# qasimyu/scssim

Hardware: AMD Instinct MI355X
Metric: paired-end read pairs/s (whole genreads job: MALBAC amplification + read allocation + read generation + FASTQ files, PE150 30x) (higher is better)
Workload: dtype u8/u32 (integer draws, byte sequences; fp64 only in the GC-weight draw and the allocation sums)

## Files before the change

include/scssim_hip.h:

```cpp
#ifndef SCSSIM_HIP_H
#define SCSSIM_HIP_H

#include <stddef.h>
#include <stdint.h>

#ifdef __cplusplus
extern "C" {
#endif

#define SCS_OK          0
#define SCS_EINVAL      1
#define SCS_EIO         2
#define SCS_EDEVICE     3
#define SCS_EOVERFLOW   4

typedef struct scs_ctx scs_ctx;

typedef struct scs_config {
    int      device;
    void*    stream;
    uint64_t seed;
    long     primers;
    double   gamma;
    double   coverage;
// ... 170 lines not shown
int         scs_profile_open(const char* profile_path, int paired, int isize, void** handle, char* errbuf, size_t errlen);
int         scs_profile_table(void* handle, int which, const uint32_t** thr, const double** cdf, size_t* n);
int         scs_profile_scalars(void* handle, double* out);
void        scs_profile_close(void* handle);

int         scs_fasta_probe(const char* fasta_path, int* n_records, uint64_t* total_bases, uint64_t* checksum,
                            char* names_buf, size_t names_len, char* errbuf, size_t errlen);
int         scs_simuvars_probe(const char* ref_fasta, const char* snp_file, const char* var_file, int* n_records, uint64_t* total_bases,
                               uint64_t* checksum, char* errbuf, size_t errlen);
int         scs_devbuf_probe(int device, uint64_t first_bytes, uint64_t second_bytes, uint64_t* caps, int* in_place);
int         scs_bgzf_probe(const void* text, uint64_t nbytes, uint32_t lds_out_cap, void* out, uint64_t cap, uint64_t* n_out);
int         scs_batch_plan_probe(uint64_t pairs, uint32_t read_length, int to_sink, int writers, int regions, int batch_shift,
                                 uint64_t* batch, uint32_t* nbatch, uint32_t* order, uint32_t* region_of, uint32_t cap);
int         scs_bgzf_device_probe(int device, const void* text, uint64_t nbytes, uint32_t zbase, void* out, uint64_t cap, uint64_t* n_out, int* guards_ok);
int         scs_scan_probe(int device, const uint32_t* in0, uint64_t n0, const uint32_t* in1, uint64_t n1, uint32_t* out0, uint32_t* out1);
int         scs_live_resources(uint64_t out[4]);
int         scs_fasta_write_index(const char* fasta_path, char* errbuf, size_t errlen);

int         scs_kernel_time(const scs_ctx* ctx, int which, const char** name, uint64_t* launches, double* ms, uint64_t* units);
int         scs_set_kernel_timing(scs_ctx* ctx, unsigned mask, unsigned every);

#ifdef __cplusplus
}
#endif
#endif
```

scssim_amd/csrc/scs_device.h:

```cpp
#pragma once
#include <stdint.h>
#include <hip/hip_runtime.h>
#include "scs_common.h"
#include "scs_simuvars.h"

namespace scs {

struct DevFrags {
    const uint64_t* goff;
    const uint32_t* len;
    const int8_t*   strand;
    const uint32_t* primers;
    uint32_t n;
    uint64_t gidx_base;
    const uint8_t* has_n;
};

struct DevAmps {
    uint32_t* parent;
    uint32_t* sl;
    uint16_t* gc;
    uint16_t* primers;
    uint64_t* uid;
    uint64_t* errs;
// ... 64 lines not shown
    int64_t  base; uint32_t flags;
    int32_t  k1;
    uint64_t e1, e2, uid;
};

void launch_attach_frags(hipStream_t s, const uint8_t* g, DevFrags fr, const uint32_t* slot_off, uint32_t* slots,
                         uint32_t* slot_tmpl, uint32_t* valid, const unsigned long long* primer_cut, uint32_t* primer_delta,
                         unsigned long long* len_part, AmplifyParams p, uint32_t t_first, uint32_t t_end, int undo, const unsigned long long* t_from);
void launch_frag_len_sum(hipStream_t s, const unsigned long long* len_part, uint32_t nf, unsigned long long* len_sum);
void launch_poisson(hipStream_t s, DevFrags fr, DevAmps semis, uint32_t n_semis, PoissonParams p, uint32_t* budget_f, uint32_t* budget_s,
                    unsigned long long* sums, unsigned long long* part, uint32_t* flags);
void launch_alloc_bpack(hipStream_t s, const double* w, const AllocPlan& pl, double* send);
void launch_alloc_bgather(hipStream_t s, const double* w, const AllocPlan& pl, const double* gathered, double* brow, int* bmap);
void launch_alloc_chunk_sum(hipStream_t s, const double* w, const double* brow, const AllocPlan& pl, double* part);
void launch_tree_sum(hipStream_t s, const double* part, uint32_t nch, double* scratch, double* total);
void launch_alloc_norm(hipStream_t s, double* w, double* brow, const int* bmap, const AllocPlan& pl, const double* total, unsigned long long reads,
                       uint32_t* rn, double* tp, uint32_t* crn, unsigned long long* sum_rn);
void launch_alloc_quota(hipStream_t s, const double* tp, uint32_t nch, unsigned long long reads, const unsigned long long* sum_rn, unsigned long long* sum_quota,
                        uint32_t* quota, double* probs, double* scratch, RngKey key);
void launch_alloc_sample(hipStream_t s, const double* w, const double* brow, const int* bmap, const AllocPlan& pl, const double* tp, const uint32_t* quota, RngKey key, uint32_t* rn);
void launch_alloc_odd_scan(hipStream_t s, const uint32_t* rn, uint32_t ac, uint32_t* odd_before, void* temp, size_t temp_bytes);
void launch_alloc_odd_counts(hipStream_t s, const uint32_t* odd_before, const AllocPlan& pl, unsigned long long* table);
void launch_alloc_parity(hipStream_t s, uint32_t* rn, const uint32_t* odd_before, uint32_t ac, const AllocPlan& pl, const unsigned long long* table);
void launch_attach_semis(hipStream_t s, const uint8_t* g, DevFrags fr, DevAmps semis, uint32_t n_semis, DevErrPool spool,
                         const uint32_t* slot_off, uint32_t* slots, uint32_t* slot_tmpl, uint32_t* valid,
                         const unsigned long long* primer_cut, uint32_t* primer_delta, AmplifyParams p, uint32_t t_first, uint32_t t_end, int undo, const unsigned long long* t_from);
uint32_t attach_dense_waves(uint32_t n_slots);
void launch_attach_plan(hipStream_t s, const uint32_t* slot_off, uint32_t nt, uint32_t n_slots, uint32_t* item_tmpl, uint32_t* wave_first, uint32_t* valid);
void launch_attach_dense(hipStream_t s, const uint8_t* g, DevFrags fr, DevAmps semis, DevErrPool spool, const uint32_t* slot_off, uint32_t* slots, const uint32_t* item_tmpl,
                         const uint32_t* wave_first, uint32_t n_slots, uint32_t* valid, const unsigned long long* primer_cut, uint32_t* primer_delta, AmplifyParams p, int undo,
                         const unsigned long long* t_from);
void launch_stock_check(hipStream_t s, const int64_t* cnt, const uint32_t* taken, unsigned long long* cut, bool from_frag, unsigned long long* info);
void launch_stock_list(hipStream_t s, const int64_t* cnt, const uint32_t* taken, uint32_t* eidx, uint32_t* etype, uint32_t* estart, unsigned long long* info);
void launch_stock_collect(hipStream_t s, const uint8_t* g, DevFrags fr, DevAmps semis, DevErrPool spool, bool from_frag, const uint32_t* slot_off, const uint32_t* slots,
                          const uint32_t* valid, const uint32_t* eidx, unsigned long long* list, unsigned long long* info, uint32_t t_first, uint32_t t_end);
// ... 148 lines not shown
```

scssim_amd/csrc/scs_k_allocate.hip:

```cpp
#include <utility>
#include <type_traits>
#include "scs_device.h"
#include "scs_seams.h"

#include <algorithm>
#include <cstdlib>
#include <cstring>
#include <rocprim/rocprim.hpp>
#include "scs_kernels_common.h"

namespace scs {

struct GcDraw { double y, r2; bool in; };
__device__ __forceinline__ GcDraw gc_attempt(uint32_t wx, uint32_t wy) {
    const double x = 2.0 * (((double)wx + 0.5) / 4294967296.0) - 1.0;
    const double y = 2.0 * (((double)wy + 0.5) / 4294967296.0) - 1.0;
    const double r2 = x * x + y * y;
    return GcDraw{y, r2, !(r2 > 1.0 || r2 == 0.0)};
}
__device__ __forceinline__ double gc_value(double mean, double sd, double y, double r2) {
    const double mult = __dsqrt_rn(-2.0 * det_log(r2) / r2);
    return mean + sd * (y * mult);
}
constexpr int WEIGHTS_BLOCK = 1024;
// ... 111 lines not shown
    double acc = 0;
    for (uint32_t i = lane; i < r.n; i += WAVE) acc += v[i];
    acc = wave_butterfly_f64(acc);
    if (lane == 0 && r.owner) part[r.c] = acc;
}
__global__ void __launch_bounds__(256) k_tree1000(const double* __restrict__ in, uint32_t n, double* __restrict__ out) {
    const uint32_t gq = blockIdx.x * 4 + (threadIdx.x >> 6), lane = threadIdx.x & 63;
    const uint32_t b = gq * ALLOC_CHUNK;
    if (b >= n) return;
    const uint32_t m = min(ALLOC_CHUNK, n - b);
    double acc = 0;
    for (uint32_t i = lane; i < m; i += WAVE) acc += in[b + i];
    acc = wave_butterfly_f64(acc);
    if (lane == 0) out[gq] = acc;
}
__global__ void __launch_bounds__(256) k_alloc_norm(double* __restrict__ w, double* __restrict__ brow, const int* __restrict__ bmap, AllocPlan pl,
                                                    const double* __restrict__ total, unsigned long long reads, uint32_t* __restrict__ rn,
                                                    double* __restrict__ tp, uint32_t* __restrict__ crn) {
    const uint32_t q = blockIdx.x * 4 + (threadIdx.x >> 6), lane = threadIdx.x & 63;
    if (q >= pl.n_interior + pl.n_boundary) return;
    const ChunkRef r = chunk_ref(pl, q);
    double* __restrict__ v = r.brow < 0 ? w + r.local0 : brow + (size_t)r.brow * ALLOC_CHUNK;
    const int* __restrict__ mp = r.brow < 0 ? nullptr : bmap + (size_t)r.brow * ALLOC_CHUNK;
    const double den = 2.2204e-16 + *total;
    double acc = 0; uint32_t cs = 0;
    for (uint32_t i = lane; i < r.n; i += WAVE) {
        const double p = v[i] / den;
        v[i] = p; acc += p;
        const uint32_t c = (uint32_t)(p * (double)(long long)reads);
        if (mp) { const int li = mp[i]; if (li >= 0) { rn[li] = c; cs += c; } }
        else { rn[r.local0 + i] = c; cs += c; }
    }
    acc = wave_butterfly_f64(acc);
    cs = wave_sum(cs);
    if (lane == 0) { if (r.owner) tp[r.c] = acc; crn[q] = cs; }
}
__global__ void __launch_bounds__(1024) k_sum_u32(const uint32_t* __restrict__ v, uint32_t n, unsigned long long* __restrict__ dst, int add) {
    __shared__ unsigned long long s_p[16];
    unsigned long long acc = 0;
    for (uint32_t i = threadIdx.x; i < n; i += blockDim.x) acc += v[i];
    acc = wave_sum_u64(acc);
    if ((threadIdx.x & 63) == 0) s_p[threadIdx.x >> 6] = acc;
    __syncthreads();
    if (threadIdx.x == 0) { unsigned long long t = 0; for (int k = 0; k < 16; ++k) t += s_p[k]; *dst = add ? *dst + t : t; }
}
__global__ void __launch_bounds__(256) k_alloc_quota(const double* __restrict__ tp, uint32_t nch, unsigned long long reads, const unsigned long long* __restrict__ sum_rn,
                                                     uint32_t* __restrict__ quota) {
    const uint32_t c = blockIdx.x * blockDim.x + threadIdx.x;
    if (c >= nch) return;
    const unsigned long long nres = reads - *sum_rn;
    quota[c] = (uint32_t)(tp[c] * (double)nres);
}
__global__ void __launch_bounds__(64) k_scan1000(const double* __restrict__ in, uint32_t n, double* __restrict__ out, double* __restrict__ last) {
    const uint32_t g = blockIdx.x, b = g * ALLOC_CHUNK, m = min(ALLOC_CHUNK, n - b), lane = threadIdx.x;
    double carry = 0;
    for (uint32_t r = 0; r < m; r += WAVE) {
        double s = r + lane < m ? in[b + r + lane] : 0.0;
#pragma unroll
        for (int d = 1; d < WAVE; d <<= 1) { const double t = shfl_up_f64(s, d); if ((int)lane >= d) s = s + t; }
// ... 10 lines not shown
__device__ __forceinline__ uint32_t first_le(const double* __restrict__ cdf, uint32_t n, double r) {
    uint32_t lo = 0, hi = n;
    while (lo < hi) { const uint32_t mid = (lo + hi) >> 1; if (r <= cdf[mid]) hi = mid; else lo = mid + 1; }
    return lo < n ? lo : n - 1;
}
__global__ void k_alloc_top_draws(const double* __restrict__ probs, uint32_t nch, unsigned long long reads, const unsigned long long* __restrict__ sum_rn,
                                  const unsigned long long* __restrict__ sum_quota, RngKey key, uint32_t* __restrict__ quota) {
    const uint32_t t = blockIdx.x * blockDim.x + threadIdx.x;
    const unsigned long long n = reads - *sum_rn - *sum_quota;
    if (t >= n) return;
    const U4 d = draw4(key, ST_ALLOC_TOP, 0, 0, t);
    const double r = 2.2204e-16 + (1 - 2.2204e-16) * ((double)d.w[0] / 4294967296.0);
    atomicAdd(&quota[first_le(probs, nch, r)], 1u);
}
__global__ void __launch_bounds__(256) k_alloc_sample(const double* __restrict__ w, const double* __restrict__ brow, const int* __restrict__ bmap, AllocPlan pl,
                                                      const double* __restrict__ tp, const uint32_t* __restrict__ quota, RngKey key, uint32_t* __restrict__ rn) {
    constexpr int ROUNDS = (ALLOC_CHUNK + WAVE - 1) / WAVE, WAVES = 4, MINE = ROUNDS / WAVES;
    static_assert(ROUNDS % WAVES == 0, "rounds of scan1000 divide among the waves");
    __shared__ double s_cdf[ALLOC_CHUNK];
    __shared__ uint32_t s_cnt[ALLOC_CHUNK];
    __shared__ double s_tot[ROUNDS];
    const uint32_t q = blockIdx.x, tid = threadIdx.x, lane = tid & 63u, wv = tid >> 6;
    const ChunkRef r = chunk_ref(pl, q);
    const uint32_t nq = quota[r.c];
    if (nq == 0) return;
    const double* __restrict__ v = r.brow < 0 ? w + r.local0 : brow + (size_t)r.brow * ALLOC_CHUNK;
    const double t = tp[r.c];
    double pv[MINE];
#pragma unroll
    for (int m = 0; m < MINE; ++m) { const uint32_t i = (uint32_t)((wv + WAVES * m) * WAVE) + lane; pv[m] = i < r.n ? v[i] : 0.0; }
#pragma unroll
    for (int m = 0; m < MINE; ++m) {
        const uint32_t k = wv + WAVES * m, i = k * WAVE + lane;
        double s = i < r.n ? pv[m] / t : 0.0;
#pragma unroll
        for (int d = 1; d < WAVE; d <<= 1) { const double u = shfl_up_f64(s, d); if ((int)lane >= d) s = s + u; }
        pv[m] = s;
        if (lane == 63) s_tot[k] = s;
    }
    __syncthreads();
#pragma unroll
    for (int m = 0; m < MINE; ++m) {
        const uint32_t k = wv + WAVES * m, i = k * WAVE + lane;
        double carry = 0;
        for (uint32_t z = 0; z < k; ++z) carry = carry + s_tot[z];
// ... 2 lines not shown
    __syncthreads();
    for (uint32_t j = tid; 4u * j < nq; j += blockDim.x) {
        const U4 d = draw4(key, ST_ALLOC_CHUNK, 0, r.c, j);
        double x[4]; uint32_t lo[4], hi[4];
#pragma unroll
        for (int i = 0; i < 4; ++i) { x[i] = 2.2204e-16 + (1 - 2.2204e-16) * ((double)d.w[i] / 4294967296.0); lo[i] = 0; hi[i] = r.n; }
        for (uint32_t span = r.n; span; span >>= 1) {
#pragma unroll
            for (int i = 0; i < 4; ++i)
                if (lo[i] < hi[i]) { const uint32_t mid = (lo[i] + hi[i]) >> 1; if (x[i] <= s_cdf[mid]) hi[i] = mid; else lo[i] = mid + 1; }
        }
#pragma unroll
        for (int i = 0; i < 4; ++i) if (4u * j + (uint32_t)i < nq) atomicAdd(&s_cnt[lo[i] < r.n ? lo[i] : r.n - 1], 1u);
    }
    __syncthreads();
    for (uint32_t i = tid; i < r.n; i += blockDim.x) {
        const uint32_t c = s_cnt[i];
        if (!c) continue;
        if (r.brow < 0) rn[r.local0 + i] += c;
        else { const int li = bmap[(size_t)r.brow * ALLOC_CHUNK + i]; if (li >= 0) rn[li] += c; }
    }
}
__global__ void k_alloc_odd_counts(const uint32_t* __restrict__ odd_before, AllocPlan pl, unsigned long long* __restrict__ table) {
    const uint32_t slot = threadIdx.x;
    if (slot >= ALLOC_SLOTS) return;
    const uint32_t n = pl.my_seg[slot].n, lo = pl.my_seg[slot].lo;
    table[(size_t)pl.my_seg[slot].order] = n ? odd_before[lo + n] - odd_before[lo] : 0u;
}
__global__ void __launch_bounds__(256) k_alloc_parity(uint32_t* __restrict__ rn, const uint32_t* __restrict__ odd_before, uint32_t ac, AllocPlan pl,
                                                      const unsigned long long* __restrict__ table) {
    __shared__ unsigned long long s_base[ALLOC_SLOTS];
    if (threadIdx.x < ALLOC_SLOTS) {
        unsigned long long b = 0;
        if (table) { const uint32_t ord = pl.my_seg[threadIdx.x].order; for (uint32_t k = 0; k < ord; ++k) b += table[k]; }
        s_base[threadIdx.x] = b;
// ... 24 lines not shown
void launch_alloc_chunk_sum(hipStream_t s, const double* w, const double* brow, const AllocPlan& pl, double* part) {
    const uint32_t nq = pl.n_interior + pl.n_boundary;
    if (nq) hipLaunchKernelGGL(k_alloc_chunk_sum, dim3(cdiv(nq, 4)), dim3(256), 0, s, w, brow, pl, part);
}
void launch_tree_sum(hipStream_t s, const double* part, uint32_t nch, double* scratch, double* total) {
    if (nch == 0) { (void)hipMemsetAsync(total, 0, 8, s); return; }
    if (nch == 1) { (void)hipMemcpyAsync(total, part, 8, hipMemcpyDeviceToDevice, s); return; }
    const double* cur = part; uint32_t n = nch; double* nxt = scratch;
    while (n > 1) {
        const uint32_t ng = cdiv(n, ALLOC_CHUNK);
        double* dst = ng == 1 ? total : nxt;
        hipLaunchKernelGGL(k_tree1000, dim3(cdiv(ng, 4)), dim3(256), 0, s, cur, n, dst);
        cur = dst; nxt += ng; n = ng;
    }
}
void launch_alloc_norm(hipStream_t s, double* w, double* brow, const int* bmap, const AllocPlan& pl, const double* total, unsigned long long reads,
                       uint32_t* rn, double* tp, uint32_t* crn, unsigned long long* sum_rn) {
    const uint32_t nq = pl.n_interior + pl.n_boundary;
    if (nq) hipLaunchKernelGGL(k_alloc_norm, dim3(cdiv(nq, 4)), dim3(256), 0, s, w, brow, bmap, pl, total, reads, rn, tp, crn);
    hipLaunchKernelGGL(k_sum_u32, dim3(1), dim3(1024), 0, s, crn, nq, sum_rn, 0);
}
static void scan_all_dev(hipStream_t s, const double* in, uint32_t n, double* out, double* scratch) {
    const uint32_t ng = cdiv(n, ALLOC_CHUNK);
    double* last = scratch; double* pre = scratch + ng;
    hipLaunchKernelGGL(k_scan1000, dim3(ng), dim3(64), 0, s, in, n, out, ng > 1 ? last : (double*)nullptr);
    if (ng == 1) return;
    scan_all_dev(s, last, ng, pre, scratch + 2 * (size_t)ng);
    hipLaunchKernelGGL(k_scan_fix, dim3(cdiv(n, 256)), dim3(256), 0, s, out, n, pre);
}
void launch_alloc_quota(hipStream_t s, const double* tp, uint32_t nch, unsigned long long reads, const unsigned long long* sum_rn, unsigned long long* sum_quota,
                        uint32_t* quota, double* probs, double* scratch, RngKey key) {
    if (nch == 0) return;
    hipLaunchKernelGGL(k_alloc_quota, dim3(cdiv(nch, 256)), dim3(256), 0, s, tp, nch, reads, sum_rn, quota);
    hipLaunchKernelGGL(k_sum_u32, dim3(1), dim3(1024), 0, s, quota, nch, sum_quota, 0);
    scan_all_dev(s, tp, nch, probs, scratch);
    hipLaunchKernelGGL(k_alloc_top_draws, dim3(cdiv((uint64_t)nch + 1024, 256)), dim3(256), 0, s, probs, nch, reads, sum_rn, sum_quota, key, quota);
}
void launch_alloc_sample(hipStream_t s, const double* w, const double* brow, const int* bmap, const AllocPlan& pl, const double* tp, const uint32_t* quota, RngKey key, uint32_t* rn) {
    const uint32_t nq = pl.n_interior + pl.n_boundary;
    if (nq) hipLaunchKernelGGL(k_alloc_sample, dim3(nq), dim3(256), 0, s, w, brow, bmap, pl, tp, quota, key, rn);
}
void launch_alloc_odd_scan(hipStream_t s, const uint32_t* rn, uint32_t ac, uint32_t* odd_before, void* temp, size_t temp_bytes) {
    (void)rocprim::exclusive_scan(temp, temp_bytes, rocprim::make_transform_iterator(rn, OddBit()), odd_before, 0u, (size_t)ac + 1, rocprim::plus<uint32_t>(), s);
}
void launch_alloc_odd_counts(hipStream_t s, const uint32_t* odd_before, const AllocPlan& pl, unsigned long long* table) {
    hipLaunchKernelGGL(k_alloc_odd_counts, dim3(1), dim3(64), 0, s, odd_before, pl, table);
}
void launch_alloc_parity(hipStream_t s, uint32_t* rn, const uint32_t* odd_before, uint32_t ac, const AllocPlan& pl, const unsigned long long* table) {
    if (ac) hipLaunchKernelGGL(k_alloc_parity, dim3(cdiv(ac, 256)), dim3(256), 0, s, rn, odd_before, ac, pl, table);
}
void launch_weights(hipStream_t s, DevAmps fulls, uint32_t n, DevTables tb, RngKey key, uint32_t frag_size, double* w) {
    if (n == 0) return;
    hipLaunchKernelGGL(k_weights, dim3(cdiv(n, (uint32_t)WEIGHTS_BLOCK)), dim3(WEIGHTS_BLOCK), 0, s, fulls, n, tb, key, frag_size, w);
}
using ScanCfg = rocprim::scan_config<256, 16, rocprim::block_load_method::block_load_transpose, rocprim::block_store_method::block_store_transpose, rocprim::block_scan_algorithm::using_warp_scan>;
// ... 38 lines not shown
```

scssim_amd/csrc/scs_k_amplify.hip:

```cpp
#include <utility>
#include <type_traits>
#include "scs_device.h"
#include "scs_seams.h"

#include <algorithm>
#include <cstdlib>
#include <cstring>
#include <rocprim/rocprim.hpp>
#include "scs_kernels_common.h"

namespace scs {
#ifdef SCS_PHASE_CLOCK
__device__ unsigned long long g_phase_att[8 * 256];
#endif
__global__ void k_amplify_init(int64_t* __restrict__ cnt, unsigned long long* __restrict__ cut, int64_t copies, uint32_t* __restrict__ delta, uint32_t* __restrict__ gdelta, uint32_t* __restrict__ flags,
                               unsigned long long* __restrict__ sums, unsigned long long nf_all, unsigned long long frag_len_all, unsigned long long total_primers,
                               uint32_t* __restrict__ pool_head_a, uint32_t* __restrict__ pool_head_b) {
    const uint32_t i = blockIdx.x * blockDim.x + threadIdx.x;
    if (i < 65536) { cnt[i] = copies; cut[i] = copies > 0 ? ~0ull : 0ull; delta[i] = 0; if (gdelta) gdelta[i] = 0; }
    if (i < SHARD_TAIL_WORDS && gdelta) gdelta[65536 + i] = 0;
    if (i < 16) sums[i] = i == DS_G_PRIMERS ? total_primers : i == DS_G_TOTALS || i == DS_G_NF ? nf_all : i == DS_G_TOTALS + 1 || i == DS_G_FRAG_LEN ? frag_len_all : i == DS_MIN_STOCK ? (unsigned long long)copies : 0ull;
    if (i == 0) { flags[0] = 0; if (pool_head_a) *pool_head_a = 0; if (pool_head_b) *pool_head_b = 0; }
}
__device__ __forceinline__ void stock_update(uint32_t i, int64_t* __restrict__ cnt, const uint32_t* __restrict__ taken, uint32_t* __restrict__ delta, unsigned long long* __restrict__ cut,
// ... 256 lines not shown
        }
        __syncthreads();
        if (!s_more) break;
    }
    if (tid == 0) {
        budget_f[t] = (uint32_t)(int)x; part[blockIdx.x] = (unsigned long long)x;
        if ((unsigned long long)x >= (1ull << 20)) atomicOr(flags, (uint32_t)FLAG_KEYSPACE);
    }
}

__global__ void __launch_bounds__(256) k_poisson(DevFrags fr, DevAmps semis, uint32_t n_cap, PoissonParams p, uint32_t* __restrict__ budget_f,
                                                 uint32_t* __restrict__ budget_s, unsigned long long* __restrict__ part, uint32_t* __restrict__ flags) {
    if (blockIdx.x < fr.n) poisson_frag_block(blockIdx.x, fr, p, budget_f, part, flags);
    else poisson_semis_block(blockIdx.x - fr.n, semis, n_cap, p, budget_s, part);
}
__global__ void __launch_bounds__(1024) k_sum_u64_add(const unsigned long long* __restrict__ v, uint32_t n, unsigned long long* __restrict__ dst) {
    __shared__ unsigned long long s_p[16];
    unsigned long long a = 0;
    for (uint32_t i = blockIdx.x * blockDim.x + threadIdx.x; i < n; i += gridDim.x * blockDim.x) a += v[i];
    a = wave_sum_u64(a);
    if ((threadIdx.x & 63) == 0) s_p[threadIdx.x >> 6] = a;
    __syncthreads();
    if (threadIdx.x == 0) { unsigned long long t = 0; for (int k = 0; k < 16; ++k) t += s_p[k]; if (t) atomicAdd(dst, t); }
}
__global__ void __launch_bounds__(1024) k_poisson_sums(const unsigned long long* __restrict__ part, uint32_t nf, uint32_t nb, unsigned long long* __restrict__ sums) {
    __shared__ unsigned long long s_p[2][16];
    unsigned long long a = 0, b = 0;
    for (uint32_t i = threadIdx.x; i < nb; i += blockDim.x) { const unsigned long long v = part[i]; if (i < nf) a += v; else b += v; }
    a = wave_sum_u64(a); b = wave_sum_u64(b);
    if ((threadIdx.x & 63) == 0) { s_p[0][threadIdx.x >> 6] = a; s_p[1][threadIdx.x >> 6] = b; }
    __syncthreads();
    if (threadIdx.x < 2) { unsigned long long t = 0; for (int k = 0; k < 16; ++k) t += s_p[threadIdx.x][k]; sums[threadIdx.x] += t; }
}

#define STOCK_KEY_BITS 46
template <bool FROM_FRAG> __device__ __forceinline__ unsigned long long attach_key(uint32_t t, uint32_t i) {
    return (((unsigned long long)t << (FROM_FRAG ? 20 : 12)) | i) + 1ull;
}
__global__ void __launch_bounds__(256) k_stock_check(const int64_t* __restrict__ cnt, const uint32_t* __restrict__ taken, unsigned long long* __restrict__ cut, int key_shift,
                                                     unsigned long long* __restrict__ info) {
    const uint32_t x = blockIdx.x * blockDim.x + threadIdx.x;
    if (x >= 65536u) return;
    const int64_t c = cnt[x]; const uint32_t d = taken[x];
    if ((int64_t)d > c) { atomicAdd(&info[0], 1ull); atomicAdd(&info[1], (unsigned long long)d); }
    else { const unsigned long long q = cut[x]; if (q != 0ull && q != ~0ull && (int64_t)d < c) { atomicAdd(&info[2], 1ull); atomicMax(&info[3], 0xFFFFFFFFull - ((q - 1ull) >> key_shift)); cut[x] = ~0ull; } }
}
__global__ void __launch_bounds__(1024) k_stock_list(const int64_t* __restrict__ cnt, const uint32_t* __restrict__ taken,
                                                     uint32_t* __restrict__ eidx, uint32_t* __restrict__ etype, uint32_t* __restrict__ estart, unsigned long long* __restrict__ info) {
// ... 354 lines not shown
    }
#ifdef SCS_PHASE_CLOCK
    __builtin_amdgcn_wave_barrier();
    if (lane < 8) atomicAdd(&g_phase_att[lane * 256 + (blockIdx.x & 255u)], lane == 7 ? 1ull : s_att_acc[lane]);
#endif
}

void launch_attach_frags(hipStream_t s, const uint8_t* g, DevFrags fr, const uint32_t* slot_off, uint32_t* slots, uint32_t* slot_tmpl,
                         uint32_t* valid, const unsigned long long* primer_cut, uint32_t* primer_delta, unsigned long long* len_part, AmplifyParams p,
                         uint32_t t_first, uint32_t t_end, int undo, const unsigned long long* t_from) {
    if (t_end <= t_first) return;
    DevAmps none{}; DevErrPool np{};
    hipLaunchKernelGGL((k_attach<true, 64>), dim3(t_end - t_first), dim3(64), 0, s, g, fr, none, 0u, np, slot_off, slots, slot_tmpl, valid, primer_cut, primer_delta, len_part, p, t_first, t_end, undo, t_from);
}
void launch_frag_len_sum(hipStream_t s, const unsigned long long* len_part, uint32_t nf, unsigned long long* len_sum) {
    if (nf) hipLaunchKernelGGL(k_sum_u64_add, dim3(std::min(cdiv(nf, 2048), 128u)), dim3(1024), 0, s, len_part, nf, len_sum);
}
void launch_poisson(hipStream_t s, DevFrags fr, DevAmps semis, uint32_t n_semis, PoissonParams p, uint32_t* budget_f, uint32_t* budget_s,
                    unsigned long long* sums, unsigned long long* part, uint32_t* flags) {
    const uint32_t semi_blocks = n_semis ? cdiv((uint64_t)n_semis + 1, 256) : 0u;
    if (fr.n + semi_blocks) {
        hipLaunchKernelGGL(k_poisson, dim3(fr.n + semi_blocks), dim3(256), 0, s, fr, semis, n_semis, p, budget_f, budget_s, part, flags);
        hipLaunchKernelGGL(k_poisson_sums, dim3(1), dim3(1024), 0, s, part, fr.n, fr.n + semi_blocks, sums);
    }
}
static int attach_semi_group(uint32_t n_semis) {
    static const int forced = seam_env("SCS_ATTACH_G") ? atoi(seam_env("SCS_ATTACH_G")) : 0;
    return forced == 2 || forced == 4 || forced == 8 || forced == 16 ? forced : (n_semis >= (1u << 18) ? 4 : 8);
}
uint32_t attach_dense_waves(uint32_t n_slots) { return n_slots / ATTACH_DENSE_STRIDE + 1u; }
void launch_attach_plan(hipStream_t s, const uint32_t* slot_off, uint32_t nt, uint32_t n_slots, uint32_t* item_tmpl, uint32_t* wave_first, uint32_t* valid) {
    hipLaunchKernelGGL(k_attach_plan, dim3(cdiv((uint64_t)nt + 1, 256)), dim3(256), 0, s, slot_off, nt, n_slots, attach_dense_waves(n_slots), item_tmpl, wave_first, valid);
}
void launch_attach_dense(hipStream_t s, const uint8_t* g, DevFrags fr, DevAmps semis, DevErrPool spool, const uint32_t* slot_off, uint32_t* slots, const uint32_t* item_tmpl,
                         const uint32_t* wave_first, uint32_t n_slots, uint32_t* valid, const unsigned long long* primer_cut, uint32_t* primer_delta, AmplifyParams p, int undo,
                         const unsigned long long* t_from) {
    const uint32_t row_words = (p.amp_max > p.amp_min ? (p.amp_max - p.amp_min) / 32u : 0u) + 2u;
    hipLaunchKernelGGL(k_attach_dense, dim3(attach_dense_waves(n_slots)), dim3(64), 0, s, g, fr, semis, spool, slot_off, slots, item_tmpl, wave_first, valid, primer_cut, primer_delta, p, 0u,
// ... 96 lines not shown
```

scssim_amd/csrc/scs_probes.cpp:

```cpp
#include "scs_ctx.h"
#include "scs_amp.h"
#include "scs_site.h"
#include "scs_support.h"

static int truth_probe(bool bam, int paired, int is_read2, uint32_t amp, uint32_t cnt, const char* rname, int n,
                       int64_t pos0, int reverse, const int32_t* events, int nev,
                       int64_t mate_pos0, int mate_reverse, const int32_t* mate_events, int mate_nev,
                       const char* seq, const char* qual, int len, const char* genome, int64_t genome_start, uint64_t genome_len,
                       char* out, size_t cap, size_t* n_out) {
    if (!rname || !seq || !qual || !genome || !n_out || n <= 0 || nev < 0 || mate_nev < 0 || (nev && !events) || (paired && mate_nev && !mate_events)) return SCS_EINVAL;
    auto pack = [](const int32_t* e, int k, std::vector<uint32_t>& v) {
        for (int i = 0; i < k; ++i) {
            if (e[3 * i] < 0 || e[3 * i] > 0xFFFF || e[3 * i + 2] <= 0 || e[3 * i + 2] > 0x7FFF) return false;
            v.push_back(tev_pack((uint32_t)e[3 * i], e[3 * i + 1] ? 1u : 0u, (uint32_t)e[3 * i + 2]));
        }
        return true;
    };
    std::vector<uint32_t> e1, e2;
    if (!pack(events, nev, e1) || (paired && !pack(mate_events, mate_nev, e2))) return SCS_EINVAL;
    TruthAln a{pos0, reverse ? 1 : 0, n, nev, e1.data(), 0, 0, 0}, m{mate_pos0, mate_reverse ? 1 : 0, n, mate_nev, e2.data(), 0, 0, 0};
    if (!truth_place(a) || a.qlen != len || (paired && !truth_place(m))) return SCS_EINVAL;
    if (a.lo < genome_start || a.hi >= genome_start + (int64_t)genome_len) return SCS_EINVAL;
    TruthLine li{amp, cnt, 0u, paired ? 1 : 0, rname, (uint32_t)strlen(rname), 0, 0, 0};
    if (paired) {
// ... 303 lines not shown
        const size_t tb = scan_temp_bytes((size_t)std::max(n0, n1));
        void* temp = (char*)mem.get(tb);
        HIP_OK(hipDeviceSynchronize());
        if (in1) exclusive_scan_u32_pair(nullptr, din[0], dout[0], n0, din[1], dout[1], n1, temp, tb);
        else exclusive_scan_u32(nullptr, din[0], dout[0], n0, temp, tb);
        probe_sync();
        for (int a = 0; a < arrays; ++a) {
            std::vector<uint32_t> h(n[a] + 1 + guard_words);
            HIP_OK(hipMemcpy(h.data(), dout[a], h.size() * 4, hipMemcpyDeviceToHost));
            for (size_t i = n[a] + 1; i < h.size(); ++i) if (h[i] != 0xA5A5A5A5u) throw ScsError(SCS_EDEVICE, "scan probe: a scan wrote behind out[n]");
            memcpy(hout[a], h.data(), (n[a] + 1) * 4);
        }
        return SCS_OK;
    } catch (const std::exception& e) { create_error() = e.what(); return SCS_EDEVICE; }
}
int scs_profile_open(const char* path, int paired, int isize, void** handle, char* errbuf, size_t errlen) {
    if (!path || !handle) return SCS_EINVAL;
    ProfileTables* T = new ProfileTables;
    try { load_profile(path, paired != 0, isize, *T); }
    catch (const std::exception& e) { copy_err(errbuf, errlen, e.what()); delete T; *handle = nullptr; return SCS_EIO; }
    *handle = T; return SCS_OK;
}
int scs_profile_table(void* handle, int which, const uint32_t** thr, const double** cdf, size_t* n) {
    if (!handle) return SCS_EINVAL;
    ProfileTables* T = (ProfileTables*)handle;
    const std::vector<uint32_t>* t; const std::vector<double>* d;
    switch (which) {
        case 0: t = &T->subs1_t; d = &T->subs1; break; case 1: t = &T->subs2_t; d = &T->subs2; break; case 2: t = &T->qual_t; d = &T->qual; break;
        case 3: t = &T->ins_t; d = &T->ins_cdf; break; case 4: t = &T->del_t; d = &T->del_cdf; break; case 5: t = &T->isize_t; d = &T->isize_cdf; break;
        case 6: if (thr) *thr = T->qual_alias.data(); if (cdf) *cdf = nullptr; if (n) *n = T->qual_alias.size(); return SCS_OK;
// ... 23 lines not shown
```

scssim_amd/csrc/scs_reads.cpp:

```cpp
#include "scs_sink.h"
#include <cerrno>

namespace scs {
void do_allocate(scs_ctx* c, uint64_t reads) {
    if (!c->amplified) throw ScsError(SCS_EINVAL, "scs_allocate_reads: call scs_amplify first");
    hipStream_t s = c->stream;
    if (reads == 0) {
        uint64_t ref_len = 0;
        for (auto& r : c->recs) { size_t p = r.name.rfind('_'); ref_len += (uint64_t)atoi(r.name.c_str() + (p == std::string::npos ? 0 : p + 1)); }
        ref_len /= 2;
        reads = (uint64_t)(ref_len * c->cfg.coverage / (long)c->prof.read_length);
    }
    if (c->cfg.verbose) fprintf(stderr, "\nNumber of reads to generate: %llu\n", (unsigned long long)reads);
    c->reads_requested = reads; c->st.reads_requested = reads;
    const uint32_t ac = c->fulls.n;
    double t0 = now_s();
    c->weights.reserve(std::max<size_t>((size_t)ac * 8, 16), s);
    c->read_numbers.reserve(((size_t)ac + 1) * 4, s); c->pair_off.reserve(((size_t)ac + 1) * 4, s);
    launch_weights(s, c->fulls.view(), ac, c->dtb, c->key, (uint32_t)c->cfg.frag_size, c->weights.as<double>());
    double* d_w = c->weights.as<double>(); uint32_t* d_rn = c->read_numbers.as<uint32_t>();

    const int R = c->cfg.shard_count, me = c->cfg.shard_rank; const bool multi = c->sharded();
    std::vector<uint64_t> segc((size_t)R * ALLOC_SLOTS, 0);
    for (auto& sg : c->full_segs) { if (sg.c < 0 || sg.c >= 5 || sg.p < 0 || sg.p >= 8) throw ScsError(SCS_EINVAL, "allocation: segment out of range"); segc[(size_t)me * ALLOC_SLOTS + sg.c * 8 + (7 - sg.p)] += sg.count; }
// ... 53 lines not shown
    AllocState* st = (AllocState*)((char*)c->dsums.p + 128);
    double* d_part = c->a_part.as<double>(); double* d_tp = c->a_tp.as<double>();
    unsigned long long* d_sum_rn = (unsigned long long*)(d_tp + nch);
    if (R > 1) {
        const size_t per = (size_t)ALLOC_SLOTS * 2 * ALLOC_CHUNK * 8;
        c->a_send.reserve(per, s); c->a_gath.reserve(per * R, s);
        launch_alloc_bpack(s, d_w, pl, c->a_send.as<double>());
        c->gather_dev(c->a_send.p, c->a_gath.p, per);
    }
    launch_alloc_bgather(s, d_w, pl, c->a_gath.as<double>(), c->a_brow.as<double>(), c->a_bmap.as<int>());
    if (multi) HIP_OK(hipMemsetAsync(d_part, 0, (size_t)nch * 8, s));
    launch_alloc_chunk_sum(s, d_w, c->a_brow.as<double>(), pl, d_part);
    if (multi) c->reduce_dev(d_part, nch, 8);
    launch_tree_sum(s, d_part, nch, c->a_scratch.as<double>(), &st->total);
    if (multi) HIP_OK(hipMemsetAsync(d_tp, 0, ((size_t)nch + 1) * 8, s));
    launch_alloc_norm(s, d_w, c->a_brow.as<double>(), c->a_bmap.as<int>(), pl, &st->total, reads, d_rn, d_tp, c->a_crn.as<uint32_t>(), d_sum_rn);
    if (multi) c->reduce_dev(d_tp, (uint64_t)nch + 1, 8);
    launch_alloc_quota(s, d_tp, nch, reads, d_sum_rn, &st->sum_quota, c->a_quota.as<uint32_t>(), c->a_probs.as<double>(), c->a_scratch.as<double>(), c->key);
    launch_alloc_sample(s, d_w, c->a_brow.as<double>(), c->a_bmap.as<int>(), pl, d_tp, c->a_quota.as<uint32_t>(), c->key, d_rn);
    if (c->cfg.paired && !multi) launch_parity_pair_offsets(s, d_rn, ac, c->pair_off.as<uint32_t>(), c->scan_tmp.p, c->scan_tmp.cap);
    else if (c->cfg.paired) {
        launch_alloc_odd_scan(s, d_rn, ac, c->odd_before.as<uint32_t>(), c->scan_tmp.p, c->scan_tmp.cap);
        unsigned long long* table = nullptr;
        if (multi) {
            c->a_odd.reserve((size_t)R * ALLOC_SLOTS * 8, s); table = c->a_odd.as<unsigned long long>();
            HIP_OK(hipMemsetAsync(table, 0, (size_t)R * ALLOC_SLOTS * 8, s));
            launch_alloc_odd_counts(s, c->odd_before.as<uint32_t>(), pl, table);
            c->reduce_dev(table, (uint64_t)R * ALLOC_SLOTS, 8);
        }
        launch_alloc_parity(s, d_rn, c->odd_before.as<uint32_t>(), ac, pl, table);
    }
    if (!c->cfg.paired || multi) launch_pair_offsets(s, d_rn, ac, c->cfg.paired != 0, c->pair_off.as<uint32_t>(), c->scan_tmp.p, c->scan_tmp.cap);
    { Mail m; m.add(ac ? (const void*)(c->pair_off.as<uint32_t>() + ac) : nullptr, 4, 0); mail_post(c, m, true); }
    mail_wait(c);
// ... 386 lines not shown
```

Measured before the change: 55.96 million.

## Defer per-amplicon read counts to sample kernel and parallelize small sum reductions

The normalization kernel no longer writes normalized weights back or scatters first-pass read counts. Instead, the sample kernel recomputes p = w/den and the floor count, then writes the final count (floor plus sampled extras) once, including for chunks with zero quota. This removes a read-modify-write pass over the read-number array and the in-place weight writeback. Separately, the single-block u32/u64 sum and poisson-sum kernels become multi-block, vectorized, atomic-accumulating reductions with a memset, which adds atomics and an extra memset per call. A probe entry point for the u64 sum is also added.

```diff
diff --git a/include/scssim_hip.h b/include/scssim_hip.h
--- a/include/scssim_hip.h
+++ b/include/scssim_hip.h
@@ -208,6 +208,7 @@
                                  uint64_t* batch, uint32_t* nbatch, uint32_t* order, uint32_t* region_of, uint32_t cap);
 int         scs_bgzf_device_probe(int device, const void* text, uint64_t nbytes, uint32_t zbase, void* out, uint64_t cap, uint64_t* n_out, int* guards_ok);
 int         scs_scan_probe(int device, const uint32_t* in0, uint64_t n0, const uint32_t* in1, uint64_t n1, uint32_t* out0, uint32_t* out1);
+int         scs_sum_u64_probe(int device, const uint64_t* v, uint64_t n, uint64_t* sum);
 int         scs_live_resources(uint64_t out[4]);
 int         scs_fasta_write_index(const char* fasta_path, char* errbuf, size_t errlen);
 
diff --git a/scssim_amd/csrc/scs_device.h b/scssim_amd/csrc/scs_device.h
--- a/scssim_amd/csrc/scs_device.h
+++ b/scssim_amd/csrc/scs_device.h
@@ -102,11 +102,13 @@
 void launch_alloc_bgather(hipStream_t s, const double* w, const AllocPlan& pl, const double* gathered, double* brow, int* bmap);
 void launch_alloc_chunk_sum(hipStream_t s, const double* w, const double* brow, const AllocPlan& pl, double* part);
 void launch_tree_sum(hipStream_t s, const double* part, uint32_t nch, double* scratch, double* total);
-void launch_alloc_norm(hipStream_t s, double* w, double* brow, const int* bmap, const AllocPlan& pl, const double* total, unsigned long long reads,
-                       uint32_t* rn, double* tp, uint32_t* crn, unsigned long long* sum_rn);
+void launch_alloc_norm(hipStream_t s, const double* w, const double* brow, const int* bmap, const AllocPlan& pl, const double* total, unsigned long long reads,
+                       double* tp, uint32_t* crn, unsigned long long* sum_rn);
 void launch_alloc_quota(hipStream_t s, const double* tp, uint32_t nch, unsigned long long reads, const unsigned long long* sum_rn, unsigned long long* sum_quota,
                         uint32_t* quota, double* probs, double* scratch, RngKey key);
-void launch_alloc_sample(hipStream_t s, const double* w, const double* brow, const int* bmap, const AllocPlan& pl, const double* tp, const uint32_t* quota, RngKey key, uint32_t* rn);
+void launch_alloc_sample(hipStream_t s, const double* w, const double* brow, const int* bmap, const AllocPlan& pl, const double* total, unsigned long long reads,
+                         const double* tp, const uint32_t* quota, RngKey key, uint32_t* rn);
+
 void launch_alloc_odd_scan(hipStream_t s, const uint32_t* rn, uint32_t ac, uint32_t* odd_before, void* temp, size_t temp_bytes);
 void launch_alloc_odd_counts(hipStream_t s, const uint32_t* odd_before, const AllocPlan& pl, unsigned long long* table);
 void launch_alloc_parity(hipStream_t s, uint32_t* rn, const uint32_t* odd_before, uint32_t ac, const AllocPlan& pl, const unsigned long long* table);
diff --git a/scssim_amd/csrc/scs_k_allocate.hip b/scssim_amd/csrc/scs_k_allocate.hip
--- a/scssim_amd/csrc/scs_k_allocate.hip
+++ b/scssim_amd/csrc/scs_k_allocate.hip
@@ -149,35 +149,44 @@
     acc = wave_butterfly_f64(acc);
     if (lane == 0) out[gq] = acc;
 }
-__global__ void __launch_bounds__(256) k_alloc_norm(double* __restrict__ w, double* __restrict__ brow, const int* __restrict__ bmap, AllocPlan pl,
-                                                    const double* __restrict__ total, unsigned long long reads, uint32_t* __restrict__ rn,
-                                                    double* __restrict__ tp, uint32_t* __restrict__ crn) {
+__device__ __forceinline__ double alloc_norm_p(double w, double den) { return w / den; }
+__device__ __forceinline__ uint32_t alloc_first_count(double p, unsigned long long reads) {
+    return (uint32_t)(p * (double)(long long)reads);
+}
+__global__ void __launch_bounds__(256) k_alloc_norm(const double* __restrict__ w, const double* __restrict__ brow, const int* __restrict__ bmap, AllocPlan pl,
+                                                    const double* __restrict__ total, unsigned long long reads, double* __restrict__ tp, uint32_t* __restrict__ crn) {
     const uint32_t q = blockIdx.x * 4 + (threadIdx.x >> 6), lane = threadIdx.x & 63;
     if (q >= pl.n_interior + pl.n_boundary) return;
     const ChunkRef r = chunk_ref(pl, q);
-    double* __restrict__ v = r.brow < 0 ? w + r.local0 : brow + (size_t)r.brow * ALLOC_CHUNK;
+    const double* __restrict__ v = r.brow < 0 ? w + r.local0 : brow + (size_t)r.brow * ALLOC_CHUNK;
     const int* __restrict__ mp = r.brow < 0 ? nullptr : bmap + (size_t)r.brow * ALLOC_CHUNK;
     const double den = 2.2204e-16 + *total;
     double acc = 0; uint32_t cs = 0;
     for (uint32_t i = lane; i < r.n; i += WAVE) {
-        const double p = v[i] / den;
-        v[i] = p; acc += p;
-        const uint32_t c = (uint32_t)(p * (double)(long long)reads);
-        if (mp) { const int li = mp[i]; if (li >= 0) { rn[li] = c; cs += c; } }
-        else { rn[r.local0 + i] = c; cs += c; }
+        const double p = alloc_norm_p(v[i], den);
+        acc += p;
+        if (!mp || mp[i] >= 0) cs += alloc_first_count(p, reads);
     }
     acc = wave_butterfly_f64(acc);
     cs = wave_sum(cs);
     if (lane == 0) { if (r.owner) tp[r.c] = acc; crn[q] = cs; }
 }
-__global__ void __launch_bounds__(1024) k_sum_u32(const uint32_t* __restrict__ v, uint32_t n, unsigned long long* __restrict__ dst, int add) {
-    __shared__ unsigned long long s_p[16];
+constexpr uint32_t SUM_U32_BLOCK = 256, SUM_U32_MAX_GRID = 1024;
+__global__ void __launch_bounds__(SUM_U32_BLOCK) k_sum_u32(const uint32_t* __restrict__ v, uint32_t n, unsigned long long* __restrict__ dst) {
+    __shared__ unsigned long long s_p[SUM_U32_BLOCK / 64];
+    const uint4* __restrict__ v4 = (const uint4*)v;
+    const uint32_t n4 = n >> 2, stride = gridDim.x * blockDim.x;
     unsigned long long acc = 0;
-    for (uint32_t i = threadIdx.x; i < n; i += blockDim.x) acc += v[i];
+    for (uint32_t i = blockIdx.x * blockDim.x + threadIdx.x; i < n4; i += stride) { const uint4 x = v4[i]; acc += (unsigned long long)x.x + x.y + x.z + x.w; }
+    if (blockIdx.x == 0 && threadIdx.x < (n & 3u)) acc += v[4u * n4 + threadIdx.x];
     acc = wave_sum_u64(acc);
     if ((threadIdx.x & 63) == 0) s_p[threadIdx.x >> 6] = acc;
     __syncthreads();
-    if (threadIdx.x == 0) { unsigned long long t = 0; for (int k = 0; k < 16; ++k) t += s_p[k]; *dst = add ? *dst + t : t; }
+    if (threadIdx.x == 0) { unsigned long long t = 0; for (uint32_t k = 0; k < SUM_U32_BLOCK / 64; ++k) t += s_p[k]; if (t) atomicAdd(dst, t); }
+}
+static void launch_sum_u32(hipStream_t s, const uint32_t* v, uint32_t n, unsigned long long* dst) {
+    (void)hipMemsetAsync(dst, 0, 8, s);
+    if (n) hipLaunchKernelGGL(k_sum_u32, dim3(std::min(cdiv(n, 4 * SUM_U32_BLOCK), SUM_U32_MAX_GRID)), dim3(SUM_U32_BLOCK), 0, s, v, n, dst);
 }
 __global__ void __launch_bounds__(256) k_alloc_quota(const double* __restrict__ tp, uint32_t nch, unsigned long long reads, const unsigned long long* __restrict__ sum_rn,
                                                      uint32_t* __restrict__ quota) {
@@ -218,7 +227,8 @@
     atomicAdd(&quota[first_le(probs, nch, r)], 1u);
 }
 __global__ void __launch_bounds__(256) k_alloc_sample(const double* __restrict__ w, const double* __restrict__ brow, const int* __restrict__ bmap, AllocPlan pl,
-                                                      const double* __restrict__ tp, const uint32_t* __restrict__ quota, RngKey key, uint32_t* __restrict__ rn) {
+                                                      const double* __restrict__ total, unsigned long long reads, const double* __restrict__ tp,
+                                                      const uint32_t* __restrict__ quota, RngKey key, uint32_t* __restrict__ rn) {
     constexpr int ROUNDS = (ALLOC_CHUNK + WAVE - 1) / WAVE, WAVES = 4, MINE = ROUNDS / WAVES;
     static_assert(ROUNDS % WAVES == 0, "rounds of scan1000 divide among the waves");
     __shared__ double s_cdf[ALLOC_CHUNK];
@@ -227,12 +237,25 @@
     const uint32_t q = blockIdx.x, tid = threadIdx.x, lane = tid & 63u, wv = tid >> 6;
     const ChunkRef r = chunk_ref(pl, q);
     const uint32_t nq = quota[r.c];
-    if (nq == 0) return;
     const double* __restrict__ v = r.brow < 0 ? w + r.local0 : brow + (size_t)r.brow * ALLOC_CHUNK;
-    const double t = tp[r.c];
+    const int* __restrict__ mp = r.brow < 0 ? nullptr : bmap + (size_t)r.brow * ALLOC_CHUNK;
+    const double t = tp[r.c], den = 2.2204e-16 + *total;
     double pv[MINE];
 #pragma unroll
     for (int m = 0; m < MINE; ++m) { const uint32_t i = (uint32_t)((wv + WAVES * m) * WAVE) + lane; pv[m] = i < r.n ? v[i] : 0.0; }
+    uint32_t first[MINE];
+#pragma unroll
+    for (int m = 0; m < MINE; ++m) { pv[m] = alloc_norm_p(pv[m], den); first[m] = alloc_first_count(pv[m], reads); }
+    if (nq == 0) {
+#pragma unroll
+        for (int m = 0; m < MINE; ++m) {
+            const uint32_t i = tid + 256u * (uint32_t)m;
+            if (i >= r.n) continue;
+            if (!mp) rn[r.local0 + i] = first[m];
+            else { const int li = mp[i]; if (li >= 0) rn[li] = first[m]; }
+        }
+        return;
+    }
 #pragma unroll
     for (int m = 0; m < MINE; ++m) {
         const uint32_t k = wv + WAVES * m, i = k * WAVE + lane;
@@ -265,11 +288,13 @@
         for (int i = 0; i < 4; ++i) if (4u * j + (uint32_t)i < nq) atomicAdd(&s_cnt[lo[i] < r.n ? lo[i] : r.n - 1], 1u);
     }
     __syncthreads();
-    for (uint32_t i = tid; i < r.n; i += blockDim.x) {
-        const uint32_t c = s_cnt[i];
-        if (!c) continue;
-        if (r.brow < 0) rn[r.local0 + i] += c;
-        else { const int li = bmap[(size_t)r.brow * ALLOC_CHUNK + i]; if (li >= 0) rn[li] += c; }
+#pragma unroll
+    for (int m = 0; m < MINE; ++m) {
+        const uint32_t i = tid + 256u * (uint32_t)m;
+        if (i >= r.n) continue;
+        const uint32_t c = first[m] + s_cnt[i];
+        if (!mp) rn[r.local0 + i] = c;
+        else { const int li = mp[i]; if (li >= 0) rn[li] = c; }
     }
 }
 __global__ void k_alloc_odd_counts(const uint32_t* __restrict__ odd_before, AllocPlan pl, unsigned long long* __restrict__ table) {
@@ -324,11 +349,11 @@
         cur = dst; nxt += ng; n = ng;
     }
 }
-void launch_alloc_norm(hipStream_t s, double* w, double* brow, const int* bmap, const AllocPlan& pl, const double* total, unsigned long long reads,
-                       uint32_t* rn, double* tp, uint32_t* crn, unsigned long long* sum_rn) {
+void launch_alloc_norm(hipStream_t s, const double* w, const double* brow, const int* bmap, const AllocPlan& pl, const double* total, unsigned long long reads,
+                       double* tp, uint32_t* crn, unsigned long long* sum_rn) {
     const uint32_t nq = pl.n_interior + pl.n_boundary;
-    if (nq) hipLaunchKernelGGL(k_alloc_norm, dim3(cdiv(nq, 4)), dim3(256), 0, s, w, brow, bmap, pl, total, reads, rn, tp, crn);
-    hipLaunchKernelGGL(k_sum_u32, dim3(1), dim3(1024), 0, s, crn, nq, sum_rn, 0);
+    if (nq) hipLaunchKernelGGL(k_alloc_norm, dim3(cdiv(nq, 4)), dim3(256), 0, s, w, brow, bmap, pl, total, reads, tp, crn);
+    launch_sum_u32(s, crn, nq, sum_rn);
 }
 static void scan_all_dev(hipStream_t s, const double* in, uint32_t n, double* out, double* scratch) {
     const uint32_t ng = cdiv(n, ALLOC_CHUNK);
@@ -342,13 +367,14 @@
                         uint32_t* quota, double* probs, double* scratch, RngKey key) {
     if (nch == 0) return;
     hipLaunchKernelGGL(k_alloc_quota, dim3(cdiv(nch, 256)), dim3(256), 0, s, tp, nch, reads, sum_rn, quota);
-    hipLaunchKernelGGL(k_sum_u32, dim3(1), dim3(1024), 0, s, quota, nch, sum_quota, 0);
+    launch_sum_u32(s, quota, nch, sum_quota);
     scan_all_dev(s, tp, nch, probs, scratch);
     hipLaunchKernelGGL(k_alloc_top_draws, dim3(cdiv((uint64_t)nch + 1024, 256)), dim3(256), 0, s, probs, nch, reads, sum_rn, sum_quota, key, quota);
 }
-void launch_alloc_sample(hipStream_t s, const double* w, const double* brow, const int* bmap, const AllocPlan& pl, const double* tp, const uint32_t* quota, RngKey key, uint32_t* rn) {
+void launch_alloc_sample(hipStream_t s, const double* w, const double* brow, const int* bmap, const AllocPlan& pl, const double* total, unsigned long long reads,
+                         const double* tp, const uint32_t* quota, RngKey key, uint32_t* rn) {
     const uint32_t nq = pl.n_interior + pl.n_boundary;
-    if (nq) hipLaunchKernelGGL(k_alloc_sample, dim3(nq), dim3(256), 0, s, w, brow, bmap, pl, tp, quota, key, rn);
+    if (nq) hipLaunchKernelGGL(k_alloc_sample, dim3(nq), dim3(256), 0, s, w, brow, bmap, pl, total, reads, tp, quota, key, rn);
 }
 void launch_alloc_odd_scan(hipStream_t s, const uint32_t* rn, uint32_t ac, uint32_t* odd_before, void* temp, size_t temp_bytes) {
     (void)rocprim::exclusive_scan(temp, temp_bytes, rocprim::make_transform_iterator(rn, OddBit()), odd_before, 0u, (size_t)ac + 1, rocprim::plus<uint32_t>(), s);
diff --git a/scssim_amd/csrc/scs_k_amplify.hip b/scssim_amd/csrc/scs_k_amplify.hip
--- a/scssim_amd/csrc/scs_k_amplify.hip
+++ b/scssim_amd/csrc/scs_k_amplify.hip
@@ -294,24 +294,37 @@
     if (blockIdx.x < fr.n) poisson_frag_block(blockIdx.x, fr, p, budget_f, part, flags);
     else poisson_semis_block(blockIdx.x - fr.n, semis, n_cap, p, budget_s, part);
 }
-__global__ void __launch_bounds__(1024) k_sum_u64_add(const unsigned long long* __restrict__ v, uint32_t n, unsigned long long* __restrict__ dst) {
-    __shared__ unsigned long long s_p[16];
-    unsigned long long a = 0;
-    for (uint32_t i = blockIdx.x * blockDim.x + threadIdx.x; i < n; i += gridDim.x * blockDim.x) a += v[i];
+constexpr uint32_t SUM_BLOCK = 256, SUM_MAX_GRID = 1024;
+__device__ __forceinline__ void sum_block_add(unsigned long long a, unsigned long long* __restrict__ dst) {
+    __shared__ unsigned long long s_p[SUM_BLOCK / 64];
     a = wave_sum_u64(a);
     if ((threadIdx.x & 63) == 0) s_p[threadIdx.x >> 6] = a;
     __syncthreads();
-    if (threadIdx.x == 0) { unsigned long long t = 0; for (int k = 0; k < 16; ++k) t += s_p[k]; if (t) atomicAdd(dst, t); }
-}
-__global__ void __launch_bounds__(1024) k_poisson_sums(const unsigned long long* __restrict__ part, uint32_t nf, uint32_t nb, unsigned long long* __restrict__ sums) {
-    __shared__ unsigned long long s_p[2][16];
+    if (threadIdx.x == 0) { unsigned long long t = 0; for (uint32_t k = 0; k < SUM_BLOCK / 64; ++k) t += s_p[k]; if (t) atomicAdd(dst, t); }
+    __syncthreads();
+}
+__global__ void __launch_bounds__(SUM_BLOCK) k_sum_u64_add(const unsigned long long* __restrict__ v, uint32_t n, unsigned long long* __restrict__ dst) {
+    const ulonglong2* __restrict__ v2 = (const ulonglong2*)v;
+    const uint32_t n2 = n >> 1, stride = gridDim.x * blockDim.x;
+    unsigned long long a = 0;
+    for (uint32_t i = blockIdx.x * blockDim.x + threadIdx.x; i < n2; i += stride) { const ulonglong2 x = v2[i]; a += x.x + x.y; }
+    if ((n & 1u) && blockIdx.x == 0 && threadIdx.x == 0) a += v[n - 1u];
+    sum_block_add(a, dst);
+}
+__global__ void __launch_bounds__(SUM_BLOCK) k_poisson_sums(const unsigned long long* __restrict__ part, uint32_t nf, uint32_t nb, unsigned long long* __restrict__ sums) {
+    const ulonglong2* __restrict__ p2 = (const ulonglong2*)part;
+    const uint32_t n2 = nb >> 1, stride = gridDim.x * blockDim.x;
     unsigned long long a = 0, b = 0;
-    for (uint32_t i = threadIdx.x; i < nb; i += blockDim.x) { const unsigned long long v = part[i]; if (i < nf) a += v; else b += v; }
-    a = wave_sum_u64(a); b = wave_sum_u64(b);
-    if ((threadIdx.x & 63) == 0) { s_p[0][threadIdx.x >> 6] = a; s_p[1][threadIdx.x >> 6] = b; }
-    __syncthreads();
-    if (threadIdx.x < 2) { unsigned long long t = 0; for (int k = 0; k < 16; ++k) t += s_p[threadIdx.x][k]; sums[threadIdx.x] += t; }
-}
+    for (uint32_t i = blockIdx.x * blockDim.x + threadIdx.x; i < n2; i += stride) {
+        const ulonglong2 x = p2[i];
+        if (2u * i < nf) a += x.x; else b += x.x;
+        if (2u * i + 1u < nf) a += x.y; else b += x.y;
+    }
+    if ((nb & 1u) && blockIdx.x == 0 && threadIdx.x == 0) { if (nb - 1u < nf) a += part[nb - 1u]; else b += part[nb - 1u]; }
+    sum_block_add(a, sums);
+    sum_block_add(b, sums + 1);
+}
+static uint32_t sum_grid(uint32_t n) { return std::min(cdiv(n, 2 * SUM_BLOCK), SUM_MAX_GRID); }
 
 #define STOCK_KEY_BITS 46
 template <bool FROM_FRAG> __device__ __forceinline__ unsigned long long attach_key(uint32_t t, uint32_t i) {
@@ -696,14 +709,14 @@
     hipLaunchKernelGGL((k_attach<true, 64>), dim3(t_end - t_first), dim3(64), 0, s, g, fr, none, 0u, np, slot_off, slots, slot_tmpl, valid, primer_cut, primer_delta, len_part, p, t_first, t_end, undo, t_from);
 }
 void launch_frag_len_sum(hipStream_t s, const unsigned long long* len_part, uint32_t nf, unsigned long long* len_sum) {
-    if (nf) hipLaunchKernelGGL(k_sum_u64_add, dim3(std::min(cdiv(nf, 2048), 128u)), dim3(1024), 0, s, len_part, nf, len_sum);
+    if (nf) hipLaunchKernelGGL(k_sum_u64_add, dim3(sum_grid(nf)), dim3(SUM_BLOCK), 0, s, len_part, nf, len_sum);
 }
 void launch_poisson(hipStream_t s, DevFrags fr, DevAmps semis, uint32_t n_semis, PoissonParams p, uint32_t* budget_f, uint32_t* budget_s,
                     unsigned long long* sums, unsigned long long* part, uint32_t* flags) {
     const uint32_t semi_blocks = n_semis ? cdiv((uint64_t)n_semis + 1, 256) : 0u;
     if (fr.n + semi_blocks) {
         hipLaunchKernelGGL(k_poisson, dim3(fr.n + semi_blocks), dim3(256), 0, s, fr, semis, n_semis, p, budget_f, budget_s, part, flags);
-        hipLaunchKernelGGL(k_poisson_sums, dim3(1), dim3(1024), 0, s, part, fr.n, fr.n + semi_blocks, sums);
+        hipLaunchKernelGGL(k_poisson_sums, dim3(sum_grid(fr.n + semi_blocks)), dim3(SUM_BLOCK), 0, s, part, fr.n, fr.n + semi_blocks, sums);
     }
 }
 static int attach_semi_group(uint32_t n_semis) {
diff --git a/scssim_amd/csrc/scs_probes.cpp b/scssim_amd/csrc/scs_probes.cpp
--- a/scssim_amd/csrc/scs_probes.cpp
+++ b/scssim_amd/csrc/scs_probes.cpp
@@ -341,6 +341,22 @@
         return SCS_OK;
     } catch (const std::exception& e) { create_error() = e.what(); return SCS_EDEVICE; }
 }
+int scs_sum_u64_probe(int device, const uint64_t* v, uint64_t n, uint64_t* sum) {
+    if ((!v && n) || !sum || n > 0x7FFFFFF0ull) return SCS_EINVAL;
+    try {
+        HIP_OK(hipSetDevice(device));
+        ProbeMem mem;
+        unsigned long long* d_v = (unsigned long long*)mem.get((n + 2) * 8); unsigned long long* d_sum = (unsigned long long*)mem.get(16);
+        HIP_OK(hipMemset(d_v, kProbeFill, (n + 2) * 8));
+        if (n) HIP_OK(hipMemcpy(d_v, v, n * 8, hipMemcpyHostToDevice));
+        HIP_OK(hipMemcpy(d_sum, sum, 8, hipMemcpyHostToDevice));
+        HIP_OK(hipDeviceSynchronize());
+        launch_frag_len_sum(nullptr, d_v, (uint32_t)n, d_sum);
+        probe_sync();
+        HIP_OK(hipMemcpy(sum, d_sum, 8, hipMemcpyDeviceToHost));
+        return SCS_OK;
+    } catch (const std::exception& e) { create_error() = e.what(); return SCS_EDEVICE; }
+}
 int scs_profile_open(const char* path, int paired, int isize, void** handle, char* errbuf, size_t errlen) {
     if (!path || !handle) return SCS_EINVAL;
     ProfileTables* T = new ProfileTables;
diff --git a/scssim_amd/csrc/scs_reads.cpp b/scssim_amd/csrc/scs_reads.cpp
--- a/scssim_amd/csrc/scs_reads.cpp
+++ b/scssim_amd/csrc/scs_reads.cpp
@@ -91,10 +91,10 @@
     if (multi) c->reduce_dev(d_part, nch, 8);
     launch_tree_sum(s, d_part, nch, c->a_scratch.as<double>(), &st->total);
     if (multi) HIP_OK(hipMemsetAsync(d_tp, 0, ((size_t)nch + 1) * 8, s));
-    launch_alloc_norm(s, d_w, c->a_brow.as<double>(), c->a_bmap.as<int>(), pl, &st->total, reads, d_rn, d_tp, c->a_crn.as<uint32_t>(), d_sum_rn);
+    launch_alloc_norm(s, d_w, c->a_brow.as<double>(), c->a_bmap.as<int>(), pl, &st->total, reads, d_tp, c->a_crn.as<uint32_t>(), d_sum_rn);
     if (multi) c->reduce_dev(d_tp, (uint64_t)nch + 1, 8);
     launch_alloc_quota(s, d_tp, nch, reads, d_sum_rn, &st->sum_quota, c->a_quota.as<uint32_t>(), c->a_probs.as<double>(), c->a_scratch.as<double>(), c->key);
-    launch_alloc_sample(s, d_w, c->a_brow.as<double>(), c->a_bmap.as<int>(), pl, d_tp, c->a_quota.as<uint32_t>(), c->key, d_rn);
+    launch_alloc_sample(s, d_w, c->a_brow.as<double>(), c->a_bmap.as<int>(), pl, &st->total, reads, d_tp, c->a_quota.as<uint32_t>(), c->key, d_rn);
     if (c->cfg.paired && !multi) launch_parity_pair_offsets(s, d_rn, ac, c->pair_off.as<uint32_t>(), c->scan_tmp.p, c->scan_tmp.cap);
     else if (c->cfg.paired) {
         launch_alloc_odd_scan(s, d_rn, ac, c->odd_before.as<uint32_t>(), c->scan_tmp.p, c->scan_tmp.cap);
```

Result: slower. 55.19 million (-1.4%).
